# Alexander-H-Liu/End-to-end-ASR-Pytorch

Hardware: AMD Instinct MI355X
Metric: audio frames/sec training (LAS+CTC, LibriSpeech 80-mel) (higher is better)
Workload: dtype f32; 1 GPU; cfg3: {"B": 32, "T": 1600, "D": 80, "V": 5000, "L": 64}; global_batch=32, parallelism=dp1

## Files before the change

### end-to-end-asr-pytorch_amd/csrc/core.cpp

```cpp
#include "common.h"
#include "knobs.h"
#include <cstdlib>
#include <mutex>
#include <vector>

namespace {
struct DevInfo {
    int cu_count = 0;
    int lds_per_cu = 0;
    bool ok = false;
};
DevInfo g_dev[64];

struct ProfRec {
    hipEvent_t a, b;
    int id;
};
bool g_prof_on = false;
std::vector<ProfRec> g_pending;
double g_total_ms[PROF_NUM];
int64_t g_launches[PROF_NUM];
std::mutex g_mu;
hipEvent_t g_cur[PROF_NUM];
}

namespace {
AsrkKnobs g_knobs;
std::once_flag g_knobs_once;
int env_int(const char *name) {
    const char *e = getenv(name);
    return e ? atoi(e) : AsrkKnobs::UNSET;
}
int env_present(const char *name) { return getenv(name) ? 1 : AsrkKnobs::UNSET; }
void read_knobs() {
    AsrkKnobs &k = g_knobs;
    k.gemm_noskinny = env_present("ASRK_GEMM_NOSKINNY");
    k.skinny_sk = env_int("ASRK_SKINNY_SK");
    k.gemm_dbg = env_int("ASRK_GEMM_DBG");
    k.gemm_nofast = env_present("ASRK_GEMM_NOFAST");
    k.split_w256 = env_int("ASRK_SPLIT_W256");
    k.split_tail = env_int("ASRK_SPLIT_TAIL");
    k.split_mfma = env_int("ASRK_SPLIT_MFMA");
    k.fwd_mt = env_int("ASRK_FWD_MT");
    k.fwd_nt = env_int("ASRK_FWD_NT");
    k.rec_bf_mt4 = env_int("ASRK_REC_BF_MT4");
    k.bwd_ub = env_int("ASRK_BWD_UB");
    k.bwd_nt = env_int("ASRK_BWD_NT");
    k.fwd_poll = env_int("ASRK_FWD_POLL");
    k.fwd_presleep = env_int("ASRK_FWD_PRESLEEP");
    k.bwd_poll = env_int("ASRK_BWD_POLL");
    k.bwd_presleep = env_int("ASRK_BWD_PRESLEEP");
    k.dbg_noload = env_present("ASRK_DBG_NOLOAD");
    k.deterministic = env_int("ASRK_DETERMINISTIC");
}
}

const AsrkKnobs &asrk_knobs_() {
    std::call_once(g_knobs_once, read_knobs);
    return g_knobs;
}

extern "C" int asrk_version(void) { return 200; }

extern "C" const char *asrk_strerror(int rc) {
    switch (rc) {
        case ASRK_OK: return "ok";
        case ASRK_EINVAL: return "asrk: invalid argument";
        case ASRK_ESHAPE: return "asrk: shape not supported by the persistent gfx950 kernels";
        case ASRK_EWORKSPACE: return "asrk: workspace too small";
        case ASRK_EDEVICE: return "asrk: device lacks the CUs/LDS the persistent kernel needs";
        case ASRK_ETIMEOUT: return "asrk: in-kernel grid synchronisation timed out";
        default: break;
    }
    if (rc > 0) return hipGetErrorString((hipError_t)rc);
    return "asrk: unknown error";
}

extern "C" int asrk_init(int device) {
    if (device < 0 || device >= 64) return ASRK_EINVAL;
    (void)asrk_knobs_();
    if (!g_dev[device].ok) {
        hipDeviceProp_t prop;
        hipError_t e = hipGetDeviceProperties(&prop, device);
        if (e != hipSuccess) return (int)e > 0 ? -(1000 + (int)e) : ASRK_EDEVICE;
        g_dev[device].cu_count = prop.multiProcessorCount;
        g_dev[device].lds_per_cu = (int)prop.maxSharedMemoryPerMultiProcessor;
        g_dev[device].ok = true;
    }
    return g_dev[device].cu_count;
}

extern "C" int asrk_cu_count_(void) {
    int dev = 0;
    if (hipGetDevice(&dev) != hipSuccess) return 0;
    if (dev < 0 || dev >= 64) return 0;
// ... 78 lines not shown
```

### end-to-end-asr-pytorch_amd/csrc/gemm.hip

```cpp
#include "common.h"
#include "knobs.h"
#include <cstdlib>
#include <algorithm>
#include <type_traits>

extern "C" int asrk_cu_count_(void);
extern "C" void asrk_prof_launches_(int id, int64_t n);
extern "C" int asrk_gemm_split_run_(int transA, int transB, int M, int N, int K, float alpha, const float *A,
                                    int lda, const float *B, int ldb, float beta, float *C, int ldc,
                                    const float *bias, const float *bias2, void *ws, int flags, hipStream_t s);

namespace {

constexpr int BM = 128, BN = 128, BK = 32;
constexpr int KC_LD = 36;
constexpr int MC_LD = 136;
constexpr int TILE_FLOATS = 4608;
constexpr int GEMM_LDS_BYTES = 4 * TILE_FLOATS * 4;

struct GemmArgs {
    const float *A, *B;
    float *C;
    const float *bias, *bias2;
    int M, N, K, lda, ldb, ldc;
    float alpha, beta;
    int splitk, k_per_split, tiles_m, tiles_n;
    int dbg;
};

template <bool KC, bool VEC>
__device__ __forceinline__ void load_tile(const float *__restrict__ P, int ld, int R, int r0,
                                          int kbase, int kend, int tid, f32x4 (&reg)[4]) {
#pragma unroll
    for (int p = 0; p < 4; ++p) {
        f32x4 v = {0.f, 0.f, 0.f, 0.f};
        if (KC) {
            const int row = r0 + (tid >> 3) + 32 * p;
            const int k = kbase + (tid & 7) * 4;
            if (row < R) {
                const float *g = P + (size_t)row * ld + k;
                if (VEC) {
                    if (k < kend) v = *reinterpret_cast<const f32x4 *>(g);
                } else {
#pragma unroll
                    for (int j = 0; j < 4; ++j)
                        if (k + j < kend) v[j] = g[j];
                }
            }
        } else {
            const int k = kbase + (tid >> 5) + 8 * p;
            const int row = r0 + (tid & 31) * 4;
            if (k < kend) {
                const float *g = P + (size_t)k * ld + row;
                if (VEC) {
                    if (row < R) v = *reinterpret_cast<const f32x4 *>(g);
                } else {
#pragma unroll
                    for (int j = 0; j < 4; ++j)
                        if (row + j < R) v[j] = g[j];
                }
            }
        }
        reg[p] = v;
// ... 667 lines not shown
                    best = cost;
                    splitk = sk;
                }
                if (tiles * sk >= 8 * slots) break;
            }
        }
    }
    if (kiters == 0) {
        splitk = 1;
        p.k_per_split = BK;
    } else {
        if (splitk > kiters) splitk = kiters;
        p.k_per_split = asrk_div_up(kiters, splitk) * BK;
        splitk = asrk_div_up(K, p.k_per_split);
    }
    p.splitk = splitk;
    if (splitk > 1) {
        p.prepass = beta == 0.f ? PRE_MEMSET : beta != 1.f ? PRE_SCALE : PRE_NONE;
        p.store = ST_ATOMIC;
    } else {
        p.prepass = PRE_NONE;
        p.store = beta != 0.f ? ST_RMW_BETA : ST_OVERWRITE;
    }
    p.vec = al_a && al_b && (lda % 4 == 0) && (ldb % 4 == 0) && ((a_kc ? K : M) % 4 == 0) &&
            ((b_kc ? K : N) % 4 == 0);
    const bool fast = p.vec && !kn.is_set(kn.gemm_nofast) && K >= 4 && (a_kc || M >= 4) && (b_kc || N >= 4);
    p.path = fast ? GEMM_FAST : GEMM_GENERIC;
    const int lds_hint = (flags >> 8) & 0xff;
    p.lds = fast ? std::min(158 * 1024, std::max(GEMM_LDS_BYTES, lds_hint * 1024)) : GEMM_LDS_BYTES;
    p.gx = tiles; p.gy = splitk; p.gz = 1;
    p.launches = 1 + (p.prepass != PRE_NONE);
    return ASRK_OK;
}

template <bool A_KC, bool B_KC>
int launch_gemm_fast(const GemmArgs &a, int lds_bytes, hipStream_t s) {
    static AsrkLdsLatch latch;
    auto kern = gemm_f32_fast_kernel<A_KC, B_KC>;
    ASRK_HIP(asrk_max_lds_once(latch, reinterpret_cast<const void *>(kern), 158 * 1024));
    dim3 grid(a.tiles_m * a.tiles_n, a.splitk, 1);
    hipLaunchKernelGGL(kern, grid, dim3(256), lds_bytes, s, a);
    ASRK_LAUNCH_CHECK();
    return ASRK_OK;
}

}

extern "C" int asrk_gemm_plan_info(int transA, int transB, int M, int N, int K, int lda, int ldb, int ldc,
                                   int align, float beta, int splitk, int flags, int ncu, int *info) {
    if (!info || ncu < 0) return ASRK_EINVAL;
    GemmPlan p;
    const int rc = gemm_plan(transA, transB, M, N, K, lda, ldb, ldc, align, beta, splitk, flags, ncu, p);
    const int rec[ASRK_GEMM_PLAN_INFO_LEN] = {p.path, p.a_kc, p.b_kc, p.vec, p.splitk, p.k_per_split, p.gx, p.gy,
                                              p.gz, p.prepass, p.store, p.lds, p.launches, p.ncu, 0, 0};
    for (int i = 0; i < ASRK_GEMM_PLAN_INFO_LEN; ++i) info[i] = rc == ASRK_OK ? rec[i] : 0;
    return rc;
}

extern "C" int asrk_gemm_f32(int transA, int transB, int M, int N, int K, float alpha,
                             const float *A, int lda, const float *B, int ldb, float beta,
                             float *C, int ldc, const float *bias, const float *bias2,
                             int splitk, int flags, void *ws, size_t ws_bytes, void *stream) {
    auto al16 = [](const void *q) { return (reinterpret_cast<uintptr_t>(q) & 15) == 0; };
    GemmPlan pl;
    const int prc = gemm_plan(transA, transB, M, N, K, lda, ldb, ldc, (al16(A) ? 1 : 0) | (al16(B) ? 2 : 0), beta,
                              splitk, flags, 0, pl);
    if (prc != ASRK_OK) return prc;
    if (pl.launches == 0) return ASRK_OK;
    if (!A || !B || !C) return ASRK_EINVAL;
    hipStream_t s = (hipStream_t)stream;
    const int prof_id = ((flags >> 8) & 0xff) > 80 ? PROF_GEMM_BG : PROF_GEMM;
    asrk_prof_work_(prof_id, 2.0 * (double)M * (double)N * (double)K);

    if (pl.path == GEMM_SPLIT) {
        if (!ws || ws_bytes < asrk_gemm_ws_bytes(M, N, K, flags)) return ASRK_EWORKSPACE;
        if ((reinterpret_cast<uintptr_t>(ws) & 15) != 0) return ASRK_EINVAL;
        asrk_prof_begin_(prof_id, s);
        const int rc = asrk_gemm_split_run_(transA, transB, M, N, K, alpha, A, lda, B, ldb, beta, C, ldc, bias,
                                            bias2, ws, flags, s);
        asrk_prof_end_(prof_id, s);
        asrk_prof_launches_(prof_id, 2);
        return rc;
    }

    if (pl.prepass == PRE_MEMSET) {
        ASRK_HIP(hipMemset2DAsync(C, (size_t)ldc * 4, 0, (size_t)N * 4, M, s));
    } else if (pl.prepass == PRE_SCALE) {
        const int64_t n = (int64_t)M * N;
        hipLaunchKernelGGL(scale_rows_kernel, dim3((unsigned)asrk_div_up64(n, 256)), dim3(256), 0, s, C, M, N, ldc,
                           beta);
        ASRK_LAUNCH_CHECK();
    }

    if (pl.path == GEMM_SKINNY_NT || pl.path == GEMM_SKINNY_NN) {
        SkinnyArgs k;
        k.A = A; k.B = B; k.C = C; k.bias = bias; k.bias2 = bias2;
        k.M = M; k.N = N; k.K = K; k.lda = lda; k.ldb = ldb; k.ldc = ldc; k.alpha = alpha;
        k.slabs = pl.tiles_n;
        k.splitk = pl.splitk;
        k.k_per_split = pl.k_per_split;
        k.overwrite = pl.store == ST_OVERWRITE ? 1 : 0;
        asrk_prof_begin_(prof_id, s);
        const dim3 grid(pl.gx, pl.gy, pl.gz);
        if (pl.path == GEMM_SKINNY_NT) hipLaunchKernelGGL(gemm_skinny_nt_kernel, grid, dim3(256), 0, s, k);
        else hipLaunchKernelGGL(gemm_skinny_nn_kernel, grid, dim3(256), 0, s, k);
        asrk_prof_end_(prof_id, s);
        ASRK_LAUNCH_CHECK();
// ... 34 lines not shown
```

### end-to-end-asr-pytorch_amd/csrc/gemm_split.hip

```cpp
#include "common.h"
#include "knobs.h"
#include <algorithm>
#include <climits>

extern "C" int asrk_cu_count_(void);

namespace {

typedef __bf16 bf16x8 __attribute__((ext_vector_type(8)));

constexpr int PIECE = 1024;

struct SplitGemmArgs {
    const unsigned char *Ap, *Bp;
    float *C;
    const float *bias, *bias2;
    int M, N, ldc;
    int KC;
    size_t rb_stride_a, rb_stride_b;
    int nk;
    int tiles_m, tiles_n;
    float alpha, beta;
    int slices, ldw;
    float *ws;
// ... 815 lines not shown
    if (!worker) return;

    const int row0 = tm * 128 + wr * 64 + 4 * (lane >> 4), col0 = tn * 256 + wc * 128 + (lane & 15);
#pragma unroll
    for (int j = 0; j < 8; ++j) {
        const int col = col0 + j * 16;
        if (col >= p.N) continue;
        float bsum = 0.f;
        if (p.bias) bsum += p.bias[col];
        if (p.bias2) bsum += p.bias2[col];
#pragma unroll
        for (int i = 0; i < 4; ++i)
#pragma unroll
            for (int r = 0; r < 4; ++r) {
                const int row = row0 + i * 16 + r;
                if (row >= p.M) continue;
                float *c = p.C + (size_t)row * p.ldc + col;
                float v = p.alpha * (j < 4 ? acc0[i][j & 3][r] : acc1[i][j & 3][r]) + bsum;
                if (p.beta != 0.f) v += p.beta * *c;
                *c = v;
            }
    }
}
#undef ASRK_P16

template <bool SK>
int launch_split_gemm_m16(const SplitGemmArgs &a, hipStream_t s) {
    constexpr int lds = 3 * 4 * 4 * 3 * PIECE;
    auto kern = gemm_bf16x6_m16_kernel<SK>;
    static AsrkLdsLatch latch;
    ASRK_HIP(asrk_max_lds_once(latch, reinterpret_cast<const void *>(kern), lds));
    hipLaunchKernelGGL(kern, dim3(a.tiles_m * a.tiles_n * (SK ? a.slices : 1)), dim3(512), lds, s, a);
    ASRK_LAUNCH_CHECK();
    if (SK) {
        const int64_t items = (int64_t)a.M * (a.ldw >> 2);
        hipLaunchKernelGGL(splitk_reduce_kernel, dim3((unsigned)asrk_div_up64(items, 256)), dim3(256), 0, s, a.ws,
                           a.slices, a.M, a.N, a.ldw, a.alpha, a.beta, a.C, a.ldc, a.bias, a.bias2);
        ASRK_LAUNCH_CHECK();
    }
    return ASRK_OK;
}

int launch_split_gemm_w256_m16(const SplitGemmArgs &a, int rb_b, hipStream_t s) {
    constexpr int lds = 4 * 6 * 2 * 3 * PIECE;
    auto kern = gemm_bf16x6_w256_m16_kernel<4>;
    static AsrkLdsLatch latch;
    ASRK_HIP(asrk_max_lds_once(latch, reinterpret_cast<const void *>(kern), lds));
    const int band = 2;
    hipLaunchKernelGGL(kern, dim3(a.tiles_m * a.tiles_n), dim3(512), lds, s, a, rb_b, band);
    ASRK_LAUNCH_CHECK();
    return ASRK_OK;
}

template <int NC, int NST, bool SPEC, int WM, bool SK = false>
int launch_split_gemm(const SplitGemmArgs &a, hipStream_t s) {
    constexpr int lds = NST * (WM + 2) * NC * 3 * PIECE;
    auto kern = gemm_bf16x6_kernel<NC, NST, SPEC, WM, SK>;
    static AsrkLdsLatch latch;
    ASRK_HIP(asrk_max_lds_once(latch, reinterpret_cast<const void *>(kern), lds));
    hipLaunchKernelGGL(kern, dim3(a.tiles_m * a.tiles_n * (SK ? a.slices : 1)), dim3(SPEC ? (WM == 2 ? 512 : 704) : 256),
                       lds, s, a);
    ASRK_LAUNCH_CHECK();
    if (SK) {
        const int64_t items = (int64_t)a.M * (a.ldw >> 2);
        hipLaunchKernelGGL(splitk_reduce_kernel, dim3((unsigned)asrk_div_up64(items, 256)), dim3(256), 0, s, a.ws,
                           a.slices, a.M, a.N, a.ldw, a.alpha, a.beta, a.C, a.ldc, a.bias, a.bias2);
        ASRK_LAUNCH_CHECK();
    }
    return ASRK_OK;
}

}

namespace {
constexpr int SPLIT_NC = 4;
constexpr int NPL = 3;
constexpr int SPLIT_MFMA16_MIN_NK = 48;

struct PanelGeom {
    int KC, rb;
    size_t rb_stride, bytes;
};
PanelGeom panel_geom(int rows, int K, bool slack = false) {
    PanelGeom g;
    g.KC = (asrk_div_up(K, 8 * SPLIT_NC) + (slack ? 1 : 0)) * SPLIT_NC;
    g.rb = asrk_div_up(rows, 128) * 2;
    g.rb_stride = (size_t)g.KC * NPL * PIECE + 4352;
    g.bytes = (size_t)g.rb * g.rb_stride;
    return g;
}

int run_split(const float *src, int ld, int rows, int K, bool trans, unsigned char *dstp, const PanelGeom &g,
              hipStream_t s) {
    const dim3 grid((unsigned)asrk_div_up64((int64_t)g.rb * (g.KC / 4), 4));
    asrk_prof_work_(PROF_SPLIT, 4.0 * (double)rows * (double)K + 6.0 * (double)g.rb * 64.0 * (double)g.KC * 8.0);
    asrk_prof_begin_(PROF_SPLIT, s);
    if (trans) {
        hipLaunchKernelGGL((split_panel_t_kernel<4>), grid, dim3(256), 0, s, src, ld, rows, K, dstp, g.KC, g.rb, g.rb_stride);
    } else {
        const bool vec = (reinterpret_cast<uintptr_t>(src) & 15) == 0 && ld % 4 == 0;
        if (vec) hipLaunchKernelGGL((split_panel_kernel<true>), grid, dim3(256), 0, s, src, ld, rows, K, dstp, g.KC, g.rb, g.rb_stride);
        else hipLaunchKernelGGL((split_panel_kernel<false>), grid, dim3(256), 0, s, src, ld, rows, K, dstp, g.KC, g.rb, g.rb_stride);
    }
    asrk_prof_end_(PROF_SPLIT, s);
    ASRK_LAUNCH_CHECK();
    return ASRK_OK;
}

int auto_slices(int M, int N, int nk) {
    if (N >= 512) return 1;
    const int ncu = asrk_cu_count_() > 0 ? asrk_cu_count_() : 256;
    const long tiles = (long)asrk_div_up(M, 128) * asrk_div_up(N, 128);
    const long want = (ncu + tiles - 1) / tiles;
    return (int)std::max(1L, std::min(want, (long)(nk / 64)));
}

int run_panel_gemm(int M, int N, int nk, float alpha, const unsigned char *Ap, size_t stride_a,
                   const unsigned char *Bp, size_t stride_b, float beta, float *C, int ldc, const float *bias,
                   const float *bias2, hipStream_t s, int slices = 1, float *ws = nullptr) {
    const AsrkKnobs &kn = asrk_knobs_();
    SplitGemmArgs a;
    a.Ap = Ap; a.Bp = Bp; a.C = C; a.bias = bias; a.bias2 = bias2;
    a.M = M; a.N = N; a.ldc = ldc; a.KC = 0; a.nk = nk; a.rb_stride_a = stride_a; a.rb_stride_b = stride_b;
    a.tiles_m = asrk_div_up(M, 128); a.tiles_n = asrk_div_up(N, 128);
    a.alpha = alpha; a.beta = beta;
    a.slices = std::min(slices, nk); a.ldw = (N + 3) & ~3; a.ws = ws;
    const bool m16 = kn.is_set(kn.split_mfma) ? kn.split_mfma == 16 : nk >= SPLIT_MFMA16_MIN_NK;
    const bool m16_sk = kn.is_set(kn.split_mfma) && kn.split_mfma == 16;
    const bool m16_128 = m16, m16_w256 = m16;
    if (a.slices > 1) return m16_sk ? launch_split_gemm_m16<true>(a, s) : launch_split_gemm<4, 3, true, 2, true>(a, s);
    const int w256 = kn.get(kn.split_w256, 1);
    if (w256 && N >= 512) {
        const int tm = asrk_div_up(M, 128), tn = asrk_div_up(N, 256);
        const int ncu = asrk_cu_count_() > 0 ? asrk_cu_count_() : 256;
        if (w256 == 2 || (long)tm * tn >= 2L * ncu) {
            SplitGemmArgs b = a;
            b.tiles_m = tm; b.tiles_n = tn; b.nk = 2 * nk;
            const long tiles = (long)tm * tn, rem = tiles % ncu;
            const int tm1 = (int)((tiles - rem) / tn);
            if (w256 == 1 && rem > 0 && rem * 10 < 6L * ncu && tm1 > 0 && tm1 < tm && kn.get(kn.split_tail, 1)) {
                b.tiles_m = tm1; b.M = tm1 * 128;
                int rc = m16_w256 ? launch_split_gemm_w256_m16(b, 2 * asrk_div_up(N, 128), s)
                                  : launch_split_gemm_w256<4, 4>(b, 2 * asrk_div_up(N, 128), s);
                if (rc != ASRK_OK) return rc;
                SplitGemmArgs c = a;
                c.Ap = a.Ap + (size_t)tm1 * 2 * a.rb_stride_a;
                c.C = a.C + (size_t)tm1 * 128 * ldc;
                c.M = M - tm1 * 128;
                c.tiles_m = asrk_div_up(c.M, 128);
                return m16_128 ? launch_split_gemm_m16<false>(c, s) : launch_split_gemm<4, 3, true, 2>(c, s);
            }
            return m16_w256 ? launch_split_gemm_w256_m16(b, 2 * asrk_div_up(N, 128), s)
                            : launch_split_gemm_w256<4, 4>(b, 2 * asrk_div_up(N, 128), s);
        }
    }
    return m16_128 ? launch_split_gemm_m16<false>(a, s) : launch_split_gemm<4, 3, true, 2>(a, s);
}
}

extern "C" size_t asrk_split_panel_stride_(int rows, int K) { return panel_geom(rows, K, true).rb_stride; }

extern "C" int asrk_gemm_takes_split(int M, int N, int K, int flags) {
    const int mode = flags & 3;
    if (mode == ASRK_GEMM_SPLIT_OFF || mode == 3 || K < 8 || M < 1 || N < 1) return 0;
    if (mode == ASRK_GEMM_SPLIT_AUTO) {
        const double hm = 2.0 * (double)M * (double)N / ((double)M + (double)N);
        const bool shallow_ok = K >= 64 && (double)M * (double)N >= 134217728.0;
        if (hm < 1500.0 || (K < 256 && !shallow_ok) || M < 256 || N < 256) return 0;
    }
    return 1;
}

extern "C" size_t asrk_gemm_ws_bytes(int M, int N, int K, int flags) {
    if (!asrk_gemm_takes_split(M, N, K, flags)) return 0;
    return panel_geom(M, K).bytes + panel_geom(N, K).bytes;
}

extern "C" int asrk_gemm_split_run_(int transA, int transB, int M, int N, int K, float alpha, const float *A,
                                    int lda, const float *B, int ldb, float beta, float *C, int ldc,
                                    const float *bias, const float *bias2, void *wsp, int flags, hipStream_t s) {
    const PanelGeom ga = panel_geom(M, K), gb = panel_geom(N, K);
    unsigned char *ws = reinterpret_cast<unsigned char *>(wsp);
    unsigned char *Ap = ws, *Bp = ws + ga.bytes;
    int rc = run_split(A, lda, M, K, transA != 0, Ap, ga, s);
    if (rc != ASRK_OK) return rc;
    rc = run_split(B, ldb, N, K, transB == 0, Bp, gb, s);
    if (rc != ASRK_OK) return rc;
    return run_panel_gemm(M, N, ga.KC / SPLIT_NC, alpha, Ap, ga.rb_stride, Bp, gb.rb_stride, beta, C, ldc, bias,
                          bias2, s);
}

extern "C" size_t asrk_split_panel_bytes(int rows, int K, int flags) {
    if (rows <= 0 || K <= 0 || flags != 0) return 0;
    return panel_geom(rows, K, true).bytes;
}

extern "C" int asrk_split_panel_f32(const float *src, int ld, int rows, int K, int trans, void *panel, int flags,
                                    void *stream) {
    if (!src || !panel || rows <= 0 || K <= 0 || ld < (trans ? rows : K) || flags != 0) return ASRK_EINVAL;
    if ((reinterpret_cast<uintptr_t>(panel) & 15) != 0) return ASRK_EINVAL;
    asrk_prof_begin_(PROF_GEMM, (hipStream_t)stream);
    const int rc = run_split(src, ld, rows, K, trans != 0, reinterpret_cast<unsigned char *>(panel),
                             panel_geom(rows, K, true), (hipStream_t)stream);
    asrk_prof_end_(PROF_GEMM, (hipStream_t)stream);
    return rc;
}

namespace {
struct PanelRange {
    const unsigned char *Ap, *Bp;
    size_t stride_a, stride_b;
    int nk;
};
int panel_range(int M, int N, int K, const void *A_panel, int a_rows, int a_K, int a_row0, int a_k0,
                const void *B_panel, int b_rows, int b_K, int b_row0, int b_k0, const float *C, int ldc, int flags,
                PanelRange &r) {
    if (M <= 0 || N <= 0 || K <= 0 || !A_panel || !B_panel || !C || ldc < N || flags != 0) return ASRK_EINVAL;
    if (a_row0 < 0 || b_row0 < 0 || a_k0 < 0 || b_k0 < 0 || a_row0 % 128 || b_row0 % 128 || a_k0 % 8 || b_k0 % 8)
        return ASRK_EINVAL;
    if (a_row0 + M > a_rows || b_row0 + N > b_rows || a_k0 + K > a_K || b_k0 + K > b_K) return ASRK_EINVAL;
    if (K % 32 != 0 && a_k0 + K != a_K && b_k0 + K != b_K) return ASRK_ESHAPE;
    const PanelGeom ga = panel_geom(a_rows, a_K, true), gb = panel_geom(b_rows, b_K, true);
    r.nk = asrk_div_up(K, 32);
    if (a_k0 / 8 + r.nk * SPLIT_NC > ga.KC || b_k0 / 8 + r.nk * SPLIT_NC > gb.KC) return ASRK_ESHAPE;
    const unsigned char *A0 = reinterpret_cast<const unsigned char *>(A_panel);
    const unsigned char *B0 = reinterpret_cast<const unsigned char *>(B_panel);
    r.Ap = A0 + (size_t)(a_row0 / 64) * ga.rb_stride + (size_t)(a_k0 / 8) * NPL * PIECE;
    r.Bp = B0 + (size_t)(b_row0 / 64) * gb.rb_stride + (size_t)(b_k0 / 8) * NPL * PIECE;
    r.stride_a = ga.rb_stride; r.stride_b = gb.rb_stride;
    return ASRK_OK;
}
}

extern "C" int asrk_gemm_panels_f32(int M, int N, int K, float alpha, const void *A_panel, int a_rows, int a_K,
                                    int a_row0, int a_k0, const void *B_panel, int b_rows, int b_K, int b_row0,
                                    int b_k0, float beta, float *C, int ldc, const float *bias,
                                    const float *bias2, int flags, void *stream) {
    PanelRange r;
    const int rc0 = panel_range(M, N, K, A_panel, a_rows, a_K, a_row0, a_k0, B_panel, b_rows, b_K, b_row0, b_k0, C, ldc,
                                flags, r);
    if (rc0 != ASRK_OK) return rc0;
    hipStream_t s = (hipStream_t)stream;
    asrk_prof_work_(PROF_GEMM, 2.0 * (double)M * (double)N * (double)K);
    asrk_prof_begin_(PROF_GEMM, s);
    const int rc = run_panel_gemm(M, N, r.nk, alpha, r.Ap, r.stride_a, r.Bp, r.stride_b, beta, C, ldc, bias, bias2, s);
    asrk_prof_end_(PROF_GEMM, s);
    return rc;
}

extern "C" size_t asrk_gemm_panels_splitk_ws_bytes(int M, int N, int splitk) {
    if (M <= 0 || N <= 0 || splitk < 0) return 0;
    const int n = splitk > 0 ? splitk : auto_slices(M, N, INT_MAX);
    return (size_t)n * (size_t)M * (size_t)((N + 3) & ~3) * sizeof(float);
}

extern "C" int asrk_gemm_panels_splitk_f32(int M, int N, int K, float alpha, const void *A_panel, int a_rows, int a_K,
                                           int a_row0, int a_k0, const void *B_panel, int b_rows, int b_K,
                                           int b_row0, int b_k0, float beta, float *C, int ldc, const float *bias,
                                           const float *bias2, int splitk, void *ws, size_t ws_bytes, int flags,
                                           void *stream) {
    if (splitk < 0 || !ws || (reinterpret_cast<uintptr_t>(ws) & 15) != 0) return ASRK_EINVAL;
    PanelRange r;
    const int rc0 = panel_range(M, N, K, A_panel, a_rows, a_K, a_row0, a_k0, B_panel, b_rows, b_K, b_row0, b_k0, C, ldc,
                                flags, r);
    if (rc0 != ASRK_OK) return rc0;
    const int slices = splitk > 0 ? splitk : auto_slices(M, N, r.nk);
    if (ws_bytes < asrk_gemm_panels_splitk_ws_bytes(M, N, slices)) return ASRK_EWORKSPACE;
    hipStream_t s = (hipStream_t)stream;
    asrk_prof_work_(PROF_GEMM, 2.0 * (double)M * (double)N * (double)K);
    asrk_prof_begin_(PROF_GEMM, s);
    const int rc = run_panel_gemm(M, N, r.nk, alpha, r.Ap, r.stride_a, r.Bp, r.stride_b, beta, C, ldc, bias, bias2, s,
                                  slices, reinterpret_cast<float *>(ws));
    asrk_prof_end_(PROF_GEMM, s);
    return rc;
}
```

### end-to-end-asr-pytorch_amd/csrc/knobs.h

```cpp
#pragma once

struct AsrkKnobs {
    static constexpr int UNSET = -0x7fffffff;
    int gemm_noskinny;
    int skinny_sk;
    int gemm_dbg;
    int gemm_nofast;
    int split_w256;
    int split_tail;
    int split_mfma;
    int fwd_mt, fwd_nt;
    int rec_bf_mt4;
    int bwd_ub, bwd_nt;
    int fwd_poll, fwd_presleep;
    int bwd_poll, bwd_presleep;
    int dbg_noload;
    int deterministic;

    int get(int v, int dflt) const { return v == UNSET ? dflt : v; }
    bool is_set(int v) const { return v != UNSET; }
};

const AsrkKnobs &asrk_knobs_();
```

### end-to-end-asr-pytorch_amd/csrc/speller.hip

```cpp
#include "common.h"
#include "knobs.h"
#include <cstdlib>

namespace {

__device__ __forceinline__ float tanh_fast(float x) {
    const float e = __expf(2.f * x);
    return 1.f - __fdividef(2.f, e + 1.f);
}
__device__ __forceinline__ float sigmoid_fast(float x) { return __fdividef(1.f, 1.f + __expf(-x)); }

unsigned long long *g_sp_dbg = nullptr;
int g_sp_dbg_slots = 0;
inline unsigned long long *sp_slot(int step, int kid) {
    const long i = (long)step * 16 + kid;
    return (g_sp_dbg && i < g_sp_dbg_slots) ? g_sp_dbg + i * 16 : nullptr;
}
#define SP_STAMP(ph)                                                                                     \
    do {                                                                                                 \
        if (p.stamps && threadIdx.x == 0) {                                                              \
            if (blockIdx.x == 0 && blockIdx.y == 0) p.stamps[ph] = __builtin_readcyclecounter();         \
            else if (blockIdx.x == gridDim.x - 1 && blockIdx.y == gridDim.y - 1 && ((ph) == 0 || (ph) == 9)) \
                p.stamps[(ph) == 0 ? 12 : 13] = __builtin_readcyclecounter();                            \
        }                                                                                                \
// ... 1318 lines not shown
        float acc = 0.f;
        for (int k = w; k < K; k += 4) {
            const float *wr = s_w + k * KW;
            const float *col = sd + k * span + sl + 2 * ks;
            for (int j = 0; j < KW; ++j) acc += col[-j] * wr[j];
        }
        part[w * 64 + sl] = acc;
        __syncthreads();
        if (tid < 64 && s0 + tid < Te)
            p.dprev[(long)b * Te + s0 + tid] = (part[tid] + part[64 + tid]) + (part[128 + tid] + part[192 + tid]);
        SP_STAMP(9);
    } else if (y < p.nT + K) {
        const int k = y - p.nT;
        float *s_dc = sm, *s_pv = sm + Te;
        float old[4];
#pragma unroll
        for (int r = 0; r < 4; ++r) {
            const int j = tid + 256 * r;
            old[r] = j < KW ? p.dWc_part[((long)b * K + k) * KW + j] : 0.f;
        }
        for (int t = tid; t < Te; t += 256) s_dc[t] = p.dconv[((long)b * Te + t) * K + k];
        for (int i = tid; i < Te + 2 * ks; i += 256) {
            const int t = i - ks;
            s_pv[i] = (t >= 0 && t < Te) ? p.prev[(long)b * p.prev_ld + t] : 0.f;
        }
        __syncthreads();
#pragma unroll
        for (int r = 0; r < 4; ++r) {
            const int j = tid + 256 * r;
            if (j < KW) {
                const float *pv = s_pv + j;
                float acc = 0.f;
                for (int t = 0; t < Te; ++t) acc += s_dc[t] * pv[t];
                p.dWc_part[((long)b * K + k) * KW + j] = old[r] + acc;
            }
        }
        for (int j = tid + 1024; j < KW; j += 256) {
            const float *pv = s_pv + j;
            float acc = 0.f;
            for (int t = 0; t < Te; ++t) acc += s_dc[t] * pv[t];
            p.dWc_part[((long)b * K + k) * KW + j] += acc;
        }
    } else {
        for (int a = tid; a < p.A; a += 256) {
            float acc = 0.f;
            for (int c = 0; c < p.TC; ++c) acc += p.dq_part[((long)b * p.TC + c) * p.A + a];
            const float qv = p.q[(long)b * p.A + a];
            p.dq_pre[(long)b * p.A + a] = acc * (1.f - qv * qv);
        }
        SP_STAMP(9);
    }
}

constexpr int DV_LC = 64;
__global__ __launch_bounds__(256) void dvalue_kernel(const float *__restrict__ attn, long attn_ld,
                                                     long attn_step, const float *__restrict__ dxh,
                                                     long step_ld, long row_ld, float *__restrict__ dvalue,
                                                     int L, int Te, int Dv) {
    extern __shared__ float s_at[];
    const int b = blockIdx.x, d = blockIdx.y * 256 + threadIdx.x;
    for (int l0 = 0; l0 < L; l0 += DV_LC) {
        const int nl = min(DV_LC, L - l0);
        __syncthreads();
        for (int i = threadIdx.x; i < nl * Te; i += 256) {
            const int l = i / Te, t = i - l * Te;
            s_at[i] = attn[(long)b * attn_ld + (long)(l0 + l) * attn_step + t];
        }
        for (int i = nl * Te + threadIdx.x; i < DV_LC * Te; i += 256) s_at[i] = 0.f;
        __syncthreads();
        if (d < Dv) {
            float g[DV_LC];
#pragma unroll
            for (int l = 0; l < DV_LC; ++l)
                g[l] = l < nl ? dxh[(long)(l0 + l) * step_ld + (long)b * row_ld + d] : 0.f;
            float *out = dvalue + (long)b * Te * Dv + d;
            for (int t = 0; t < Te; ++t) {
                float acc = 0.f;
#pragma unroll
                for (int l = 0; l < DV_LC; ++l) acc += s_at[l * Te + t] * g[l];
                if (l0 == 0) out[(long)t * Dv] = acc;
                else out[(long)t * Dv] += acc;
            }
        }
    }
}

__global__ __launch_bounds__(256) void joint_score_kernel(const float *__restrict__ att,
                                                          const int64_t *__restrict__ cand,
                                                          const float *__restrict__ psi,
                                                          const float *__restrict__ prev_ctc,
                                                          const float *__restrict__ lm, float *__restrict__ out,
                                                          int V, int C, float wa, float w_ctc, float w_lm,
                                                          float logzero) {
    const int r = blockIdx.x;
    const float *a = att + (long)r * V;
    const float *l = lm ? lm + (long)r * V : nullptr;
    float *o = out + (long)r * V;
    const bool ctc = cand != nullptr;
    const float wz = w_ctc * logzero;
    for (int v = threadIdx.x; v < V; v += 256) {
        float x = a[v];
        if (ctc) x = (v == 0) ? logzero : wa * x + wz;
        if (l) x = x + w_lm * l[v];
        o[v] = x;
    }
    if (!ctc) return;
    __syncthreads();
    for (int c = threadIdx.x; c < C; c += 256) {
        const int v = (int)cand[(long)r * C + c];
        if (v <= 0 || v >= V) continue;
        float x = wa * a[v] + w_ctc * (psi[(long)r * C + c] - prev_ctc[r]);
        if (l) x = x + w_lm * l[v];
        o[v] = x;
    }
}

__global__ __launch_bounds__(256) void transpose_ld_kernel(const float *__restrict__ in, long ldi,
                                                           float *__restrict__ out, long ldo, int rows,
                                                           int cols) {
    __shared__ float tile[32][33];
    const int tx = threadIdx.x & 31, ty = threadIdx.x >> 5;
    const int c0 = blockIdx.x * 32, r0 = blockIdx.y * 32;
    for (int i = ty; i < 32; i += 8)
        if (r0 + i < rows && c0 + tx < cols) tile[i][tx] = in[(long)(r0 + i) * ldi + c0 + tx];
    __syncthreads();
    for (int i = ty; i < 32; i += 8)
        if (c0 + i < cols && r0 + tx < rows) out[(long)(c0 + i) * ldo + r0 + tx] = tile[tx][i];
}

int pick_tpb(int B, int Te, int A, int K, size_t fixed_floats, size_t per_frame_floats, size_t budget, int wg_target = 512) {
    int tc = asrk_div_up(wg_target, B > 0 ? B : 1);
    if (tc > asrk_div_up(Te, 8)) tc = asrk_div_up(Te, 8);
    if (tc < 1) tc = 1;
    int tpb = asrk_div_up(Te, tc);
// ... 77 lines not shown

int check_dims(const asrk_speller_t *d) {
    if (!d) return ASRK_EINVAL;
    if (d->B < 0 || d->Te <= 0 || d->A <= 0 || d->Dv <= 0 || (d->K <= 0 && d->att_mode == 0) || d->K < 0 ||
        d->ks < 0 || d->H <= 0 || d->E < 0 || d->L < 0 || d->temperature == 0.f)
        return ASRK_EINVAL;
    if (d->nlayer < 0 || d->nlayer > ASRK_SPELLER_MAX_LAYERS || (d->nlayer > 1 && d->cell != 0)) return ASRK_ESHAPE;
    if (d->att_mode != 0 && d->att_mode != 1) return ASRK_EINVAL;
    if (d->nhead < 0 || (d->nhead > 1 && d->att_mode != 1) || (d->att_mode == 1 && d->A > 64 * DOT_NA)) return ASRK_ESHAPE;
    return ASRK_OK;
}

inline int n_layers(const asrk_speller_t &d) { return d.nlayer > 1 ? d.nlayer : 1; }
inline int n_heads(const asrk_speller_t &d) { return d.nhead > 1 ? d.nhead : 1; }
inline float *h_of(const asrk_speller_t &d, int l) { return l == 0 ? d.h : d.hu[l - 1]; }
inline float *c_of(const asrk_speller_t &d, int l) { return l == 0 ? d.c : d.cu[l - 1]; }
inline float *g_of(const asrk_speller_t &d, int l) { return l == 0 ? d.gates : d.gu[l - 1]; }
inline bool upper_ok(const asrk_speller_t &d, bool fwd) {
    for (int l = 1; l < n_layers(d); ++l)
        if (!d.Wu_ih[l - 1] || !d.Wu_hh[l - 1] || !d.hu[l - 1] || !d.cu[l - 1] || !d.gu[l - 1] ||
            (fwd && (!d.bu_ih[l - 1] || !d.bu_hh[l - 1])))
            return false;
    return true;
}

template <typename T>
int set_lds(T kernel, size_t bytes) {
    ASRK_HIP(hipFuncSetAttribute(reinterpret_cast<const void *>(kernel),
                                 hipFuncAttributeMaxDynamicSharedMemorySize, (int)bytes));
    return ASRK_OK;
}

}

extern "C" void asrk_prof_launches_(int id, int64_t n);

extern "C" int asrk_transpose_ld_f32(const float *in, int64_t ldi, float *out, int64_t ldo, int rows,
                                     int cols, void *stream) {
    if (rows < 0 || cols < 0 || ldi < cols || ldo < rows) return ASRK_EINVAL;
    if (rows == 0 || cols == 0) return ASRK_OK;
    if (!in || !out) return ASRK_EINVAL;
    hipLaunchKernelGGL(transpose_ld_kernel, dim3(asrk_div_up(cols, 32), asrk_div_up(rows, 32)), dim3(256), 0,
                       (hipStream_t)stream, in, (long)ldi, out, (long)ldo, rows, cols);
    ASRK_LAUNCH_CHECK();
    return ASRK_OK;
}

extern "C" int asrk_speller_dvalue_f32(const float *attn, int64_t attn_ld, int64_t attn_step, const float *dxh,
                                       int64_t step_ld, int64_t row_ld, float *dvalue, int B, int L, int Te,
                                       int Dv, void *stream) {
    if (B < 0 || L <= 0 || Te <= 0 || Dv <= 0) return ASRK_EINVAL;
    if (B == 0) return ASRK_OK;
    if (!attn || !dxh || !dvalue) return ASRK_EINVAL;
    const size_t lds = (size_t)DV_LC * Te * sizeof(float);
    if (lds > LDS_BUDGET) return ASRK_ESHAPE;
    int rc = set_lds(dvalue_kernel, lds);
    if (rc) return rc;
    hipLaunchKernelGGL(dvalue_kernel, dim3(B, asrk_div_up(Dv, 256)), dim3(256), lds, (hipStream_t)stream, attn,
                       (long)attn_ld, (long)attn_step, dxh, (long)step_ld, (long)row_ld, dvalue, L, Te, Dv);
    ASRK_LAUNCH_CHECK();
    return ASRK_OK;
}

extern "C" void asrk_speller_set_debug_(void *buf, int slots) {
    g_sp_dbg = reinterpret_cast<unsigned long long *>(buf);
    g_sp_dbg_slots = slots;
}

extern "C" int asrk_speller_plan(const asrk_speller_t *d, int *tc_fwd, int *tc_bwd) {
    int rc = check_dims(d);
    if (rc) return rc;
    Plan pl;
    rc = make_plan(*d, pl);
    if (rc) return rc;
    if (tc_fwd) *tc_fwd = pl.tc_f;
    if (tc_bwd) *tc_bwd = pl.tc_b;
    return ASRK_OK;
}

extern "C" int asrk_speller_plan_info(const asrk_speller_t *d, int *info) {
    if (!info) return ASRK_EINVAL;
    int rc = check_dims(d);
    if (rc) return rc;
    Plan pl;
    rc = make_plan(*d, pl);
    if (rc) return rc;
    const int v[8] = {pl.ae2_na, pl.ae2_km, pl.eb3_na, pl.eb3_km, pl.tpb_f, pl.tpb_b, pl.KP, d->Dv % 4 == 0};
    for (int i = 0; i < 8; ++i) info[i] = v[i];
    return ASRK_OK;
}

enum { CTX_SCALAR = 0, CTX_VECTOR = 1, CTX_GROUP = 2 };
static int ctx_variant(const asrk_speller_t &d, const float *ctxh_t) {
    const bool vec = al16(d.value) && d.Dv % 4 == 0;
    const int RG = d.row_group;
    const size_t lds_g = (size_t)RG * ((d.Te + 3) & ~3) * sizeof(float);
    if (RG > 1 && RG <= 8 * CG_MAXR && n_heads(d) == 1 && vec && d.B % RG == 0 && al16(ctxh_t) && d.Dv % 4 == 0 &&
        lds_g <= 64 * 1024 && !d.shared_kv && (d.B / RG) * asrk_div_up(d.Dv, 256) >= 64)
        return CTX_GROUP;
    return vec ? CTX_VECTOR : CTX_SCALAR;
}

extern "C" int asrk_speller_ctx_variant(const asrk_speller_t *d, int *variant) {
    if (!variant) return ASRK_EINVAL;
    int rc = check_dims(d);
    if (rc) return rc;
    if (d->row_group < 0) return ASRK_EINVAL;
    *variant = ctx_variant(*d, n_heads(*d) > 1 ? d->ctxh : d->ctx);
    return ASRK_OK;
}

// ... 359 lines not shown
```

Baseline: 544,000 frames/s.

## Add short-K bf16x6 GEMM kernel and MFMA-based speller dvalue kernel

Adds a small-K GEMM path that keeps the whole A fragment in registers. It streams B tiles through LDS with register prefetch and splits N into chunks so enough blocks exist, and it is taken by default when K/16 is at most 8. Separately, the speller dvalue backward kernel is rewritten from a scalar LDS-staged outer product to fp32 MFMA 32x32x2 tiles. That version also parallelises over time chunks in grid z and needs no LDS. Both aim to cut time in small-K GEMMs and the attention value gradient, at the cost of new code paths and less reuse of loads across l.

```diff
diff --git a/end-to-end-asr-pytorch_amd/csrc/core.cpp b/end-to-end-asr-pytorch_amd/csrc/core.cpp
--- a/end-to-end-asr-pytorch_amd/csrc/core.cpp
+++ b/end-to-end-asr-pytorch_amd/csrc/core.cpp
@@ -41,6 +41,7 @@
     k.split_w256 = env_int("ASRK_SPLIT_W256");
     k.split_tail = env_int("ASRK_SPLIT_TAIL");
     k.split_mfma = env_int("ASRK_SPLIT_MFMA");
+    k.split_think = env_int("ASRK_SPLIT_THINK");
     k.fwd_mt = env_int("ASRK_FWD_MT");
     k.fwd_nt = env_int("ASRK_FWD_NT");
     k.rec_bf_mt4 = env_int("ASRK_REC_BF_MT4");
diff --git a/end-to-end-asr-pytorch_amd/csrc/gemm.hip b/end-to-end-asr-pytorch_amd/csrc/gemm.hip
--- a/end-to-end-asr-pytorch_amd/csrc/gemm.hip
+++ b/end-to-end-asr-pytorch_amd/csrc/gemm.hip
@@ -9,6 +9,7 @@
 extern "C" int asrk_gemm_split_run_(int transA, int transB, int M, int N, int K, float alpha, const float *A,
                                     int lda, const float *B, int ldb, float beta, float *C, int ldc,
                                     const float *bias, const float *bias2, void *ws, int flags, hipStream_t s);
+extern "C" int asrk_gemm_split_kernel_(int K);
 
 namespace {
 
@@ -782,7 +783,8 @@
     GemmPlan p;
     const int rc = gemm_plan(transA, transB, M, N, K, lda, ldb, ldc, align, beta, splitk, flags, ncu, p);
     const int rec[ASRK_GEMM_PLAN_INFO_LEN] = {p.path, p.a_kc, p.b_kc, p.vec, p.splitk, p.k_per_split, p.gx, p.gy,
-                                              p.gz, p.prepass, p.store, p.lds, p.launches, p.ncu, 0, 0};
+                                              p.gz, p.prepass, p.store, p.lds, p.launches, p.ncu,
+                                              p.path == GEMM_SPLIT ? asrk_gemm_split_kernel_(K) : 0, 0};
     for (int i = 0; i < ASRK_GEMM_PLAN_INFO_LEN; ++i) info[i] = rc == ASRK_OK ? rec[i] : 0;
     return rc;
 }
diff --git a/end-to-end-asr-pytorch_amd/csrc/gemm_split.hip b/end-to-end-asr-pytorch_amd/csrc/gemm_split.hip
--- a/end-to-end-asr-pytorch_amd/csrc/gemm_split.hip
+++ b/end-to-end-asr-pytorch_amd/csrc/gemm_split.hip
@@ -891,6 +891,118 @@
     return ASRK_OK;
 }
 
+constexpr int THINK_MAX_STEPS = 8;
+constexpr int THINK_CHUNK_TILES = 16;
+
+template <int NS>
+__global__ __launch_bounds__(256) void gemm_bf16x6_think_kernel(SplitGemmArgs p, int nchunks, int chunk_tiles) {
+    constexpr int NPL = 3, HALF = PIECE / 2;
+    constexpr int ITEMS = NS * 2 * NPL * 32;
+    constexpr int NQ = (ITEMS + 255) / 256;
+    __shared__ __attribute__((aligned(16))) unsigned char bt[ITEMS * 16];
+    const int tid = threadIdx.x, lane = tid & 63, r = lane & 31, h = lane >> 5;
+    const int wave = __builtin_amdgcn_readfirstlane(tid >> 6);
+    const int rblk = blockIdx.x / nchunks, chunk = blockIdx.x - rblk * nchunks;
+    const int nt0 = chunk * chunk_tiles, nt1 = min(nt0 + chunk_tiles, (p.N + 31) >> 5);
+
+    bf16x8 fa[NS][NPL];
+    {
+        const unsigned char *ap = p.Ap + (size_t)(rblk * 2 + (wave >> 1)) * p.rb_stride_a + (wave & 1) * HALF +
+                                  h * NPL * PIECE + r * 16;
+#pragma unroll
+        for (int s = 0; s < NS; ++s)
+#pragma unroll
+            for (int pl = 0; pl < NPL; ++pl)
+                fa[s][pl] = *reinterpret_cast<const bf16x8 *>(ap + (s * 2 * NPL + pl) * PIECE);
+    }
+
+    u32x4 pf[NQ];
+    auto prefetch = [&](int nt) __attribute__((always_inline)) {
+        const unsigned char *bp = p.Bp + (size_t)(nt >> 1) * p.rb_stride_b + (nt & 1) * HALF;
+#pragma unroll
+        for (int q = 0; q < NQ; ++q) {
+            const int i = tid + q * 256;
+            if (ITEMS % 256 == 0 || i < ITEMS)
+                pf[q] = *reinterpret_cast<const u32x4 *>(bp + (size_t)(i >> 5) * PIECE + (i & 31) * 16);
+        }
+    };
+    const int row0 = rblk * 128 + wave * 32 + 4 * h;
+    const bool rows_live = rblk * 128 + wave * 32 < p.M;
+    const unsigned char *bfrag = bt + h * NPL * HALF + r * 16;
+    constexpr int PA[6] = {2, 1, 0, 1, 0, 0};
+    constexpr int PB[6] = {0, 1, 2, 0, 1, 0};
+
+    if (nt0 < nt1) prefetch(nt0);
+    for (int nt = nt0; nt < nt1; ++nt) {
+#pragma unroll
+        for (int q = 0; q < NQ; ++q) {
+            const int i = tid + q * 256;
+            if (ITEMS % 256 == 0 || i < ITEMS) *reinterpret_cast<u32x4 *>(bt + i * 16) = pf[q];
+        }
+        __syncthreads();
+        if (nt + 1 < nt1) prefetch(nt + 1);
+        if (rows_live) {
+            f32x16 acc;
+#pragma unroll
+            for (int e = 0; e < 16; ++e) acc[e] = 0.f;
+#pragma unroll
+            for (int s = 0; s < NS; ++s) {
+                bf16x8 fb[NPL];
+#pragma unroll
+                for (int pl = 0; pl < NPL; ++pl)
+                    fb[pl] = *reinterpret_cast<const bf16x8 *>(bfrag + (s * 2 * NPL + pl) * HALF);
+#pragma unroll
+                for (int t = 0; t < 6; ++t)
+                    acc = __builtin_amdgcn_mfma_f32_32x32x16_bf16(fa[s][PA[t]], fb[PB[t]], acc, 0, 0, 0);
+            }
+            const int col = nt * 32 + r;
+            if (col < p.N) {
+                float bsum = 0.f;
+                if (p.bias) bsum += p.bias[col];
+                if (p.bias2) bsum += p.bias2[col];
+#pragma unroll
+                for (int e = 0; e < 16; ++e) {
+                    const int row = row0 + (e & 3) + 8 * (e >> 2);
+                    if (row >= p.M) continue;
+                    float *c = p.C + (size_t)row * p.ldc + col;
+                    float v = p.alpha * acc[e] + bsum;
+                    if (p.beta != 0.f) v += p.beta * *c;
+                    *c = v;
+                }
+            }
+        }
+        __syncthreads();
+    }
+}
+
+template <int NS>
+int launch_think_ns(const SplitGemmArgs &a, int nchunks, int chunk_tiles, hipStream_t s) {
+    hipLaunchKernelGGL(gemm_bf16x6_think_kernel<NS>, dim3((unsigned)(a.tiles_m * nchunks)), dim3(256), 0, s, a, nchunks,
+                       chunk_tiles);
+    ASRK_LAUNCH_CHECK();
+    return ASRK_OK;
+}
+
+int launch_split_gemm_think(const SplitGemmArgs &a, int nk16, hipStream_t s) {
+    const int ncu = asrk_cu_count_() > 0 ? asrk_cu_count_() : 256;
+    const int tn32 = asrk_div_up(a.N, 32);
+    int ct = THINK_CHUNK_TILES;
+    while (ct > 1 && (long)a.tiles_m * asrk_div_up(tn32, ct) < 4L * ncu) ct >>= 1;
+    const int nchunks = asrk_div_up(tn32, ct);
+    if ((long)a.tiles_m * nchunks > INT_MAX) return ASRK_ESHAPE;
+    switch (nk16) {
+        case 1: return launch_think_ns<1>(a, nchunks, ct, s);
+        case 2: return launch_think_ns<2>(a, nchunks, ct, s);
+        case 3: return launch_think_ns<3>(a, nchunks, ct, s);
+        case 4: return launch_think_ns<4>(a, nchunks, ct, s);
+        case 5: return launch_think_ns<5>(a, nchunks, ct, s);
+        case 6: return launch_think_ns<6>(a, nchunks, ct, s);
+        case 7: return launch_think_ns<7>(a, nchunks, ct, s);
+        case 8: return launch_think_ns<8>(a, nchunks, ct, s);
+        default: return ASRK_ESHAPE;
+    }
+}
+
 template <int NC, int NST, bool SPEC, int WM, bool SK = false>
 int launch_split_gemm(const SplitGemmArgs &a, hipStream_t s) {
     constexpr int lds = NST * (WM + 2) * NC * 3 * PIECE;
@@ -915,6 +1027,7 @@
 constexpr int SPLIT_NC = 4;
 constexpr int NPL = 3;
 constexpr int SPLIT_MFMA16_MIN_NK = 48;
+constexpr int SPLIT_THINK_MAX_NK16 = 8;
 
 struct PanelGeom {
     int KC, rb;
@@ -954,10 +1067,18 @@
     return (int)std::max(1L, std::min(want, (long)(nk / 64)));
 }
 
+bool takes_think(int nk16) {
+    const AsrkKnobs &kn = asrk_knobs_();
+    if (nk16 < 1 || nk16 > THINK_MAX_STEPS) return false;
+    if (kn.is_set(kn.split_think)) return kn.split_think != 0;
+    return nk16 <= SPLIT_THINK_MAX_NK16 && kn.get(kn.split_mfma, 32) != 16;
+}
+
 int run_panel_gemm(int M, int N, int nk, float alpha, const unsigned char *Ap, size_t stride_a,
                    const unsigned char *Bp, size_t stride_b, float beta, float *C, int ldc, const float *bias,
-                   const float *bias2, hipStream_t s, int slices = 1, float *ws = nullptr) {
+                   const float *bias2, hipStream_t s, int slices = 1, float *ws = nullptr, int nk16 = 0) {
     const AsrkKnobs &kn = asrk_knobs_();
+    if (nk16 <= 0 || nk16 > 2 * nk) nk16 = 2 * nk;
     SplitGemmArgs a;
     a.Ap = Ap; a.Bp = Bp; a.C = C; a.bias = bias; a.bias2 = bias2;
     a.M = M; a.N = N; a.ldc = ldc; a.KC = 0; a.nk = nk; a.rb_stride_a = stride_a; a.rb_stride_b = stride_b;
@@ -968,6 +1089,7 @@
     const bool m16_sk = kn.is_set(kn.split_mfma) && kn.split_mfma == 16;
     const bool m16_128 = m16, m16_w256 = m16;
     if (a.slices > 1) return m16_sk ? launch_split_gemm_m16<true>(a, s) : launch_split_gemm<4, 3, true, 2, true>(a, s);
+    if (takes_think(nk16)) return launch_split_gemm_think(a, nk16, s);
     const int w256 = kn.get(kn.split_w256, 1);
     if (w256 && N >= 512) {
         const int tm = asrk_div_up(M, 128), tn = asrk_div_up(N, 256);
@@ -1010,6 +1132,8 @@
     return 1;
 }
 
+extern "C" int asrk_gemm_split_kernel_(int K) { return K > 0 && takes_think(asrk_div_up(K, 16)) ? 1 : 0; }
+
 extern "C" size_t asrk_gemm_ws_bytes(int M, int N, int K, int flags) {
     if (!asrk_gemm_takes_split(M, N, K, flags)) return 0;
     return panel_geom(M, K).bytes + panel_geom(N, K).bytes;
@@ -1026,7 +1150,7 @@
     rc = run_split(B, ldb, N, K, transB == 0, Bp, gb, s);
     if (rc != ASRK_OK) return rc;
     return run_panel_gemm(M, N, ga.KC / SPLIT_NC, alpha, Ap, ga.rb_stride, Bp, gb.rb_stride, beta, C, ldc, bias,
-                          bias2, s);
+                          bias2, s, 1, nullptr, asrk_div_up(K, 16));
 }
 
 extern "C" size_t asrk_split_panel_bytes(int rows, int K, int flags) {
@@ -1082,7 +1206,8 @@
     hipStream_t s = (hipStream_t)stream;
     asrk_prof_work_(PROF_GEMM, 2.0 * (double)M * (double)N * (double)K);
     asrk_prof_begin_(PROF_GEMM, s);
-    const int rc = run_panel_gemm(M, N, r.nk, alpha, r.Ap, r.stride_a, r.Bp, r.stride_b, beta, C, ldc, bias, bias2, s);
+    const int rc = run_panel_gemm(M, N, r.nk, alpha, r.Ap, r.stride_a, r.Bp, r.stride_b, beta, C, ldc, bias, bias2, s, 1,
+                                  nullptr, asrk_div_up(K, 16));
     asrk_prof_end_(PROF_GEMM, s);
     return rc;
 }
diff --git a/end-to-end-asr-pytorch_amd/csrc/knobs.h b/end-to-end-asr-pytorch_amd/csrc/knobs.h
--- a/end-to-end-asr-pytorch_amd/csrc/knobs.h
+++ b/end-to-end-asr-pytorch_amd/csrc/knobs.h
@@ -9,6 +9,7 @@
     int split_w256;
     int split_tail;
     int split_mfma;
+    int split_think;
     int fwd_mt, fwd_nt;
     int rec_bf_mt4;
     int bwd_ub, bwd_nt;
diff --git a/end-to-end-asr-pytorch_amd/csrc/speller.hip b/end-to-end-asr-pytorch_amd/csrc/speller.hip
--- a/end-to-end-asr-pytorch_amd/csrc/speller.hip
+++ b/end-to-end-asr-pytorch_amd/csrc/speller.hip
@@ -1394,34 +1394,39 @@
     }
 }
 
-constexpr int DV_LC = 64;
+constexpr int DV_LC = 16, DV_COLS = 128;
 __global__ __launch_bounds__(256) void dvalue_kernel(const float *__restrict__ attn, long attn_ld,
                                                      long attn_step, const float *__restrict__ dxh,
                                                      long step_ld, long row_ld, float *__restrict__ dvalue,
                                                      int L, int Te, int Dv) {
-    extern __shared__ float s_at[];
-    const int b = blockIdx.x, d = blockIdx.y * 256 + threadIdx.x;
-    for (int l0 = 0; l0 < L; l0 += DV_LC) {
-        const int nl = min(DV_LC, L - l0);
-        __syncthreads();
-        for (int i = threadIdx.x; i < nl * Te; i += 256) {
-            const int l = i / Te, t = i - l * Te;
-            s_at[i] = attn[(long)b * attn_ld + (long)(l0 + l) * attn_step + t];
-        }
-        for (int i = nl * Te + threadIdx.x; i < DV_LC * Te; i += 256) s_at[i] = 0.f;
-        __syncthreads();
-        if (d < Dv) {
-            float g[DV_LC];
-#pragma unroll
-            for (int l = 0; l < DV_LC; ++l)
-                g[l] = l < nl ? dxh[(long)(l0 + l) * step_ld + (long)b * row_ld + d] : 0.f;
-            float *out = dvalue + (long)b * Te * Dv + d;
-            for (int t = 0; t < Te; ++t) {
-                float acc = 0.f;
-#pragma unroll
-                for (int l = 0; l < DV_LC; ++l) acc += s_at[l * Te + t] * g[l];
-                if (l0 == 0) out[(long)t * Dv] = acc;
-                else out[(long)t * Dv] += acc;
+    const int lane = threadIdx.x & 63, j = lane & 31, h = lane >> 5;
+    const int b = blockIdx.x, d = blockIdx.y * DV_COLS + (threadIdx.x >> 6) * 32 + j;
+    const bool d_ok = d < Dv;
+    const float *gp = dxh + (long)b * row_ld + min(d, Dv - 1);
+    for (int t0 = blockIdx.z * 32; t0 < Te; t0 += gridDim.z * 32) {
+        const bool t_ok = t0 + j < Te;
+        const float *ap = attn + (long)b * attn_ld + min(t0 + j, Te - 1);
+        f32x16 acc;
+#pragma unroll
+        for (int r = 0; r < 16; ++r) acc[r] = 0.f;
+        for (int l0 = 0; l0 < L; l0 += DV_LC) {
+            float a[DV_LC / 2], g[DV_LC / 2];
+#pragma unroll
+            for (int s = 0; s < DV_LC / 2; ++s) {
+                const int l = l0 + 2 * s + h, lc = min(l, L - 1);
+                const float av = ap[(long)lc * attn_step], gv = gp[(long)lc * step_ld];
+                a[s] = (t_ok && l < L) ? av : 0.f;
+                g[s] = (d_ok && l < L) ? gv : 0.f;
+            }
+#pragma unroll
+            for (int s = 0; s < DV_LC / 2; ++s) acc = __builtin_amdgcn_mfma_f32_32x32x2f32(a[s], g[s], acc, 0, 0, 0);
+        }
+        if (d_ok) {
+            float *out = dvalue + ((long)b * Te + t0) * Dv + d;
+#pragma unroll
+            for (int r = 0; r < 16; ++r) {
+                const int t = (r & 3) + 8 * (r >> 2) + 4 * h;
+                if (t0 + t < Te) out[(long)t * Dv] = acc[r];
             }
         }
     }
@@ -1605,11 +1610,11 @@
     if (B < 0 || L <= 0 || Te <= 0 || Dv <= 0) return ASRK_EINVAL;
     if (B == 0) return ASRK_OK;
     if (!attn || !dxh || !dvalue) return ASRK_EINVAL;
-    const size_t lds = (size_t)DV_LC * Te * sizeof(float);
-    if (lds > LDS_BUDGET) return ASRK_ESHAPE;
-    int rc = set_lds(dvalue_kernel, lds);
-    if (rc) return rc;
-    hipLaunchKernelGGL(dvalue_kernel, dim3(B, asrk_div_up(Dv, 256)), dim3(256), lds, (hipStream_t)stream, attn,
+    const int ny = asrk_div_up(Dv, DV_COLS), nt = asrk_div_up(Te, 32);
+    if (ny > 65535) return ASRK_ESHAPE;
+    const long xy = (long)B * ny;
+    const int tz = (int)std::min<long>(nt, std::max<long>(1, (2048 + xy - 1) / xy));
+    hipLaunchKernelGGL(dvalue_kernel, dim3(B, ny, tz), dim3(256), 0, (hipStream_t)stream, attn,
                        (long)attn_ld, (long)attn_step, dxh, (long)step_ld, (long)row_ld, dvalue, L, Te, Dv);
     ASRK_LAUNCH_CHECK();
     return ASRK_OK;
```

Measured after the change: 549,300 frames/s, median of 6. Within noise of the previous version (+1.0%).
